# ajingu/RealSenseCalibration

Hardware: AMD Instinct MI355X
Metric: LM iterations/sec (64 cams x 100k pts point model; + final reprojection RMS px) (higher is better)
Workload: dtype f64

## Files before the change

realsensecalibration_amd/csrc/ba_schur_plan.hpp:

```cpp
#pragma once
#include <algorithm>
#include <climits>
#include <cstddef>
#include <cstdint>
#include <vector>

namespace rsba {

#define RSBA_TG 16
#define RSBA_MAX_STAGES 32
#ifndef RSBA_CHUNK
#define RSBA_CHUNK 512
#endif
#define RSBA_CW (RSBA_CHUNK / 64)
#define RSBA_GRP 8
#define RSBA_GRP_SMALL 4
#define RSBA_SELF_SETS 6
#define RSBA_DIRECT_GROUPS 4
#define RSBA_HIT_NONE 0xffffffffu
#define RSBA_CHOL_MAXN 384
#define RSBA_PB 32
#define RSBA_PLD (RSBA_PB + 1)
#define RSBA_CT 64
#define RSBA_BSM_BPG 3
// ... 20 lines not shown
    for (int I = J + 2; I < nrt && (int)first.size() < extra; ++I) { first.push_back(I << 8 | J); taken[(size_t)I * nrt + J] = 1; }
  for (int J = nrt - 1; J >= 0 && (int)last.size() < (int)first.size(); --J)
    for (int I = nrt - 1; I >= J && (int)last.size() < (int)first.size(); --I)
      if (!taken[(size_t)I * nrt + J]) { last.push_back(I << 8 | J); taken[(size_t)I * nrt + J] = 1; }
  order = first;
  for (int I = 0; I < nrt; ++I) for (int J = 0; J <= I; ++J) if (!taken[(size_t)I * nrt + J]) order.push_back(I << 8 | J);
  order.insert(order.end(), last.begin(), last.end());
  return order;
}

struct SchurSeg {
  int ga, gb, word_begin, word_end, self;
  int tile, grp, grp_seg0, grp_nseg, tile_grp0, tile_ngrp, stage, stage_ntiles, nred, index, pad2;
};

struct SchurPlanSwitches {
  static constexpr int kUnset = INT_MIN;
  int seg_per_cu = kUnset;
  int seg_target = kUnset;
  bool sparse_pairs = true;
  int balance = 1;
  bool balance_parity = true;
  int red_delay = 250;
  static SchurPlanSwitches FromEnv();
};

struct PointLayout {
  std::vector<int> ptr;
  std::vector<int> cam;
  std::vector<double> u, v;
// ... 39 lines not shown
```

realsensecalibration_amd/csrc/ba_schur_tiled.hpp:

```cpp
#pragma once
#include <type_traits>
#include <hip/hip_runtime.h>

#include <vector>

#include "ba_point_kernels.hpp"
#include "ba_schur_plan.hpp"

struct rsba_solver;

namespace rsba {

class KernelTimer;

#define RSBA_READY_ALLDIAG 40
#define RSBA_READY_SOLVED 41
#define RSBA_READY_STARTED 42
#define RSBA_PRIO(p) __builtin_amdgcn_s_setprio(p)
#ifndef RSBA_RESIDENT
#define RSBA_RESIDENT 0
#endif
#if RSBA_RESIDENT
#define RSBA_PRIO_HITS(stage) do { if ((stage) == 0) RSBA_PRIO(2); else if ((stage) == 1) RSBA_PRIO(1); else RSBA_PRIO(0); } while (0)
#else
// ... 30 lines not shown
  int ntiles = 0;
  double* ptdata = nullptr;
  double* partial = nullptr;
  double* grp_sum = nullptr;
  int* tree_error = nullptr;
  int self_arrivals = 0;
  int* error_flag = nullptr;
  int* grp_flag = nullptr;
  int epoch = 0;
  int* sync_cnt = nullptr;
  int nsync = 0, nblocks = 0;
  int* ready = nullptr;
  int* block_seg = nullptr;
  SchurSeg* segs_ordered = nullptr;
  unsigned ticket_base = 0;
  SchurSeg* segs_ordered_self = nullptr;
  int* small_flag = nullptr;
  int nblocks_self = 0;
  int ngrp = 0;
  double* block_scal = nullptr;
  int* cam_prefix = nullptr;
  int* cam_ptr = nullptr;
  int* cm_pos = nullptr;
  double* sq_cm2[2] = {nullptr, nullptr};
  double* lin2[2] = {nullptr, nullptr};
  bool has_first_order = false;
  SchurSeg* segs_ordered_first = nullptr;
  bool lin_valid = false;
  bool pt_valid = false;
  int pt_state = -1, scal_blocks = 0;
// ... 304 lines not shown
      for (int i = 0; i < NV; ++i) v[i] = (v[i] + x0[i]) + x1[i];
    }
  }
  for (; q < n; ++q) {
    const double* p0 = in + (size_t)q * RSBA_PART * 256;
#pragma unroll
    for (int i = 0; i < NV; ++i) v[i] += p0[i * 256];
  }
}

__device__ __forceinline__ bool SingleSegmentGroup(const SchurSeg& sg) { return sg.grp_nseg == 1 && sg.nred != 0; }
__device__ __forceinline__ double* SegmentOut(const SchurSeg& sg, double* __restrict__ partial, double* __restrict__ grp_sum, int seg_index) {
  return SingleSegmentGroup(sg) ? grp_sum + (size_t)sg.grp * RSBA_PART * 256 : partial + (size_t)seg_index * RSBA_PART * 256;
}

template <int NV>
__device__ __forceinline__ bool GroupReduce(const SchurSeg& sg, const double* __restrict__ partial, double* __restrict__ grp_sum,
                                            int* __restrict__ sync_cnt, int ngrp, double* v, int* __restrict__ grp_flag, int epoch) {
  __shared__ int s_last;
  const int tid = OpaqueTid();
  __builtin_amdgcn_s_waitcnt(0);
  __syncthreads();
  if (SingleSegmentGroup(sg)) {
    if (tid == 0) __hip_atomic_store(&grp_flag[sg.grp], epoch, __ATOMIC_RELAXED, __HIP_MEMORY_SCOPE_AGENT);
    return false;
  }
  if (tid == 0) s_last = __hip_atomic_fetch_add(&sync_cnt[sg.grp], 1, __ATOMIC_RELAXED, __HIP_MEMORY_SCOPE_AGENT) == sg.grp_nseg - 1;
  __syncthreads();
  if (!s_last) return false;
  __builtin_amdgcn_fence(__ATOMIC_ACQUIRE, "agent");
  TreeSum<NV>(partial + (size_t)sg.grp_seg0 * RSBA_PART * 256 + tid, sg.grp_nseg, v);
  double* gs = grp_sum + (size_t)sg.grp * RSBA_PART * 256 + tid;
#pragma unroll
  for (int i = 0; i < NV; ++i) __hip_atomic_store(&gs[i * 256], v[i], __ATOMIC_RELAXED, __HIP_MEMORY_SCOPE_AGENT);
  if (tid == 0) __hip_atomic_store(&sync_cnt[sg.grp], 0, __ATOMIC_RELAXED, __HIP_MEMORY_SCOPE_AGENT);
  __builtin_amdgcn_s_waitcnt(0);
  __syncthreads();
  if (tid == 0) {
    __hip_atomic_store(&grp_flag[sg.grp], epoch, __ATOMIC_RELAXED, __HIP_MEMORY_SCOPE_AGENT);
    s_last = sg.nred == 0 && __hip_atomic_fetch_add(&sync_cnt[ngrp + sg.tile], 1, __ATOMIC_RELAXED, __HIP_MEMORY_SCOPE_AGENT) == sg.tile_ngrp - 1;
  }
  __syncthreads();
  if (sg.nred != 0 || !s_last) return false;
  if (tid == 0) __hip_atomic_store(&sync_cnt[ngrp + sg.tile], 0, __ATOMIC_RELAXED, __HIP_MEMORY_SCOPE_AGENT);
// ... 176 lines not shown
  const double* __restrict__ block_scal;
  double* __restrict__ gmax_p;
  int* tree_error;
  int* ticket;
  unsigned ticket_base;
  int total;
  int* grp_flag;
  int epoch;
  long long* trace;
  long long* wg_trace;
  const unsigned* __restrict__ hits;
  const unsigned* __restrict__ hit_off;
  const int* __restrict__ hit_trips;
};

template <bool kLoss, bool kSmall>
__device__ __forceinline__ void PairSegment(const SchurArgs& a, const SchurSeg& sg, int seg_index, int ticket, double* pt, unsigned long long (*mk)[RSBA_CW], double* sc) {
  const int C = a.C, P = a.P, nwords = a.nwords;
  const double* __restrict__ camc = a.camc;
  const unsigned long long* __restrict__ cam_mask = a.cam_mask;
  const double* __restrict__ ptdata = a.ptdata;
  const int* __restrict__ cam_prefix = a.cam_prefix;
  const int* __restrict__ cam_ptr = a.cam_ptr;
  const double* __restrict__ sq_cm = a.sq_cm;
  double* __restrict__ partial = a.partial;
  const int tid = OpaqueTid();
  const bool diag_tile = sg.ga == sg.gb;
  const int dt = diag_tile ? (tid & 127) : tid;
  const int pr = diag_tile ? (dt < 120 ? kDiagPair[dt] : 0) : tid;
  const int ia = pr >> 4, ib = pr & 15;
  const int cam_a = RSBA_TG * sg.ga + ia, cam_b = RSBA_TG * sg.gb + ib;
  const bool live = cam_a < C && cam_b < C && (!diag_tile || dt < 120);
  const int w0 = diag_tile ? (tid >> 7) : 0, wstep = diag_tile ? 2 : 1;
  double scv[2];
#pragma unroll
  for (int u = 0; u < 2; ++u) {
    const int i = tid + 256 * u;
    const int row = i / RSBA_SC_STRIDE, e = i - row * RSBA_SC_STRIDE;
    const int cam = row < RSBA_TG ? RSBA_TG * sg.ga + row : RSBA_TG * sg.gb + (row - RSBA_TG);
    const double* cc = camc + (size_t)(cam < C ? cam : 0) * CC_STRIDE;
    const int src = e < 9 ? CC_R + e : (e < 12 ? CC_T + e - 9 : (e == 12 ? CC_FX : (e == 13 ? CC_FY : CC_SMALL)));
    scv[u] = e < 15 ? cc[src] : 0.0;
  }
  const double* ca = sc + ia * RSBA_SC_STRIDE;
  const double* cb = sc + (RSBA_TG + ib) * RSBA_SC_STRIDE;
  {
    const int wb = sg.word_begin;
    const int nwc = min(RSBA_CW, sg.word_end - wb);
    const int j0 = wb * 64;
    const int np = max(0, min(nwc * 64, P - j0));
    static_assert(RSBA_PT_STRIDE == 12, "six 16-byte pieces a record");
    constexpr int kPtPerThread = RSBA_CHUNK * 6 / 256;
    double2 pv[kPtPerThread];
    const double2* __restrict__ src2 = reinterpret_cast<const double2*>(ptdata + (size_t)j0 * RSBA_PT_STRIDE);
#pragma unroll
    for (int u = 0; u < kPtPerThread; ++u) { const int i = tid + 256 * u; pv[u] = i < np * 6 ? src2[i] : make_double2(0.0, 0.0); }
    unsigned long long mv;
    {
      const int row = tid >> 3, w = tid & 7;
      const int cam = row < RSBA_TG ? RSBA_TG * sg.ga + row : RSBA_TG * sg.gb + (row - RSBA_TG);
      mv = (cam < C && w < nwc) ? cam_mask[(size_t)cam * nwords + (size_t)wb + w] : 0ull;
    }
    sc[tid] = scv[0]; sc[tid + 256] = scv[1];
    PtLdsCursor pc(tid);
#pragma unroll
    for (int u = 0; u < kPtPerThread; ++u) { const int i = tid + 256 * u; if (i < np * 6) reinterpret_cast<double2*>(pt)[pc.a] = pv[u]; pc.Next(); }
    if ((tid & 7) < RSBA_CW) mk[tid >> 3][tid & 7] = mv;
    __syncthreads();
  }
  double acc[36];
#pragma unroll
  for (int i = 0; i < 36; ++i) acc[i] = 0.0;

  for (int wb = sg.word_begin; wb < sg.word_end; wb += RSBA_CW) {
    const int nwc = min(RSBA_CW, sg.word_end - wb);
    if (wb != sg.word_begin) {
      const int j0 = wb * 64;
      const int np = max(0, min(nwc * 64, P - j0));
      __syncthreads();
      { PtLdsCursor pc(tid); const double2* __restrict__ src2 = reinterpret_cast<const double2*>(ptdata + (size_t)j0 * RSBA_PT_STRIDE);
        for (int i = tid; i < np * 6; i += 256) { reinterpret_cast<double2*>(pt)[pc.a] = src2[i]; pc.Next(); } }
      {
// ... 28 lines not shown
    RSBA_PRIO(3);
  }
  if (diag_tile) {
    __syncthreads();
    if (tid >= 128 && dt < 120) {
#pragma unroll
      for (int i = 0; i < 36; ++i) pt[i * 128 + dt] = acc[i];
    }
    __syncthreads();
    if (tid < 120) {
#pragma unroll
      for (int i = 0; i < 36; ++i) acc[i] += pt[i * 128 + tid];
    }
  }
  double* out = SegmentOut(sg, partial, a.grp_sum, seg_index);
  if (!diag_tile || tid < 120) {
#pragma unroll
    for (int i = 0; i < 36; ++i) __hip_atomic_store(&out[i * 256 + pr], acc[i], __ATOMIC_RELAXED, __HIP_MEMORY_SCOPE_AGENT);
  }
  if (a.wg_trace && tid == 0) a.wg_trace[3 * ticket + 2] = wall_clock64();
  double v[36];
  if (!GroupReduce<36>(sg, partial, a.grp_sum, a.sync_cnt, a.ngrp, v, a.grp_flag, a.epoch)) return;
  FinishPairSlot(C, sg.ga, sg.gb, tid, v, camc, a.red, a.L, a.cam_free);
  if (!StageArrive(sg, a.sync_cnt, a.ngrp, a.ntiles, a.tag != 0)) return;
  if (tid == 0 && a.tag) PublishStage(a.ready + 1 + sg.stage, a.tag);
  if (a.trace && tid == 0 && sg.stage < 7) a.trace[17 + sg.stage] = wall_clock64();
}

template <bool kLoss, bool kSmall>
__device__ __forceinline__ void PairSegmentSparse(const SchurArgs& a, const SchurSeg& sg, int seg_index, int ticket, double* pt, double* sc) {
  const int C = a.C;
  const double* __restrict__ camc = a.camc;
  const double* __restrict__ ptdata = a.ptdata;
  const double* __restrict__ sq_cm = a.sq_cm;
  double* __restrict__ partial = a.partial;
// ... 56 lines not shown
      for (int i = 0; i < 36; ++i) pt[i * 128 + dt] = acc[i];
    }
    __syncthreads();
    if (tid < 120) {
#pragma unroll
      for (int i = 0; i < 36; ++i) acc[i] += pt[i * 128 + tid];
    }
  }
  double* out = SegmentOut(sg, partial, a.grp_sum, seg_index);
  if (!diag_tile || tid < 120) {
#pragma unroll
    for (int i = 0; i < 36; ++i) __hip_atomic_store(&out[i * 256 + pr], acc[i], __ATOMIC_RELAXED, __HIP_MEMORY_SCOPE_AGENT);
  }
  if (a.wg_trace && tid == 0) a.wg_trace[3 * ticket + 2] = wall_clock64();
  double v[36];
  if (!GroupReduce<36>(sg, partial, a.grp_sum, a.sync_cnt, a.ngrp, v, a.grp_flag, a.epoch)) return;
  FinishPairSlot(C, sg.ga, sg.gb, tid, v, camc, a.red, a.L, a.cam_free);
  if (!StageArrive(sg, a.sync_cnt, a.ngrp, a.ntiles, a.tag != 0)) return;
  if (tid == 0 && a.tag) PublishStage(a.ready + 1 + sg.stage, a.tag);
  if (a.trace && tid == 0 && sg.stage < 7) a.trace[17 + sg.stage] = wall_clock64();
}

template <bool kLoss>
__device__ __forceinline__ void SelfSegment(const SchurArgs& a, const SchurSeg& sg, int seg_index, int ticket, double* pt, unsigned long long (*mk)[RSBA_CW],
                                            unsigned short (*lst)[RSBA_CHUNK], int* cnt) {
  const int C = a.C, P = a.P, nwords = a.nwords;
  const double* __restrict__ camc = a.camc;
  const unsigned long long* __restrict__ cam_mask = a.cam_mask;
  const double* __restrict__ ptdata = a.ptdata;
  const int* __restrict__ cam_prefix = a.cam_prefix;
  const int* __restrict__ cam_ptr = a.cam_ptr;
  const double* __restrict__ sq_cm = a.sq_cm;
  const double* __restrict__ u_cm = a.u_cm;
  const double* __restrict__ v_cm = a.v_cm;
  double* __restrict__ partial = a.partial;
  const int tid = OpaqueTid(), ia = tid >> 4, ib = tid & 15;
  const int cam_a = RSBA_TG * sg.ga + ia;
  const bool live = cam_a < C;
  const double* cca = camc + (size_t)(live ? cam_a : 0) * CC_STRIDE;
  SideConst A;
  LoadSide(cca, A);
  const double ppx = cca[CC_PPX], ppy = cca[CC_PPY];
  const int obs0 = live ? cam_ptr[cam_a] : 0;
  double acc[RSBA_PART];
#pragma unroll
  for (int i = 0; i < RSBA_PART; ++i) acc[i] = 0.0;
  for (int wb = sg.word_begin; wb < sg.word_end; wb += RSBA_CW) {
    const int nwc = min(RSBA_CW, sg.word_end - wb);
    const int j0 = wb * 64;
    const int np = max(0, min(nwc * 64, P - j0));
    static_assert(RSBA_PT_STRIDE == 12, "six 16-byte pieces a record");
    constexpr int kPtPerThread = RSBA_CHUNK * 6 / 256;
    double2 pv[kPtPerThread];
    const double2* __restrict__ src2 = reinterpret_cast<const double2*>(ptdata + (size_t)j0 * RSBA_PT_STRIDE);
#pragma unroll
    for (int u = 0; u < kPtPerThread; ++u) { const int i = tid + 256 * u; pv[u] = i < np * 6 ? src2[i] : make_double2(0.0, 0.0); }
    unsigned long long mv = 0ull;
    if (tid < RSBA_TG * 8) {
      const int row = tid >> 3, w = tid & 7;
      const int cam = RSBA_TG * sg.ga + row;
      mv = (cam < C && w < nwc) ? cam_mask[(size_t)cam * nwords + (size_t)wb + w] : 0ull;
    }
    const int obs_chunk_pre = live ? cam_prefix[(size_t)cam_a * nwords + wb] : 0;
    __syncthreads();
    PtLdsCursor pc(tid);
#pragma unroll
    for (int u = 0; u < kPtPerThread; ++u) { const int i = tid + 256 * u; if (i < np * 6) reinterpret_cast<double2*>(pt)[pc.a] = pv[u]; pc.Next(); }
    if (tid < RSBA_TG * 8 && (tid & 7) < RSBA_CW) mk[tid >> 3][tid & 7] = mv;
    __syncthreads();
    {
      const int row = tid >> 4, j = tid & 15, w = j >> 1, half = j & 1;
      int base = 0;
#pragma unroll
      for (int x = 0; x < RSBA_CW; ++x) base += x < w ? __popcll(mk[row][x]) : 0;
      const unsigned long long m = w < RSBA_CW ? mk[row][w] : 0ull;
      unsigned int my = half ? (unsigned int)(m >> 32) : (unsigned int)m;
      if (half) base += __popc((unsigned int)m);
      if (j == 2 * RSBA_CW - 1) cnt[row] = base + __popc(my);
      const int p0 = w * 64 + half * 32;
      while (my != 0u) {
        const int b = __ffs((int)my) - 1;
        my &= my - 1u;
        lst[row][base++] = (unsigned short)(p0 + b);
// ... 37 lines not shown
        }
      }
      acc[21] = Fma2(e0[0], e0[0], e1[0], e1[0], acc[21]); acc[22] = Fma2(e0[0], e0[1], e1[0], e1[1], acc[22]); acc[23] = Fma2(e0[0], e0[2], e1[0], e1[2], acc[23]);
      acc[24] = Fma2(e0[1], e0[1], e1[1], e1[1], acc[24]); acc[25] = Fma2(e0[1], e0[2], e1[1], e1[2], acc[25]); acc[26] = Fma2(e0[2], e0[2], e1[2], e1[2], acc[26]);
      acc[27] = fma(e0[3], e0[3], acc[27]); acc[28] = fma(e1[4], e1[4], acc[28]); acc[29] = Fma2(e0[5], e0[5], e1[5], e1[5], acc[29]);
      const double f0 = n0[0] * pd[9] + n0[1] * pd[10] + n0[2] * pd[11];
      const double f1 = n1[0] * pd[9] + n1[1] * pd[10] + n1[2] * pd[11];
#pragma unroll
      for (int p = 0; p < 6; ++p) {
        if (p == 3) { acc[33] = fma(e0[3], r0, acc[33]); acc[39] = fma(e0[3], f0, acc[39]); }
        else if (p == 4) { acc[34] = fma(e1[4], r1, acc[34]); acc[40] = fma(e1[4], f1, acc[40]); }
        else { acc[30 + p] = Fma2(e0[p], r0, e1[p], r1, acc[30 + p]); acc[36 + p] = Fma2(e0[p], f0, e1[p], f1, acc[36 + p]); }
      }
    }
    RSBA_PRIO(3);
  }
  double* out = SegmentOut(sg, partial, a.grp_sum, seg_index);
#pragma unroll
  for (int i = 0; i < RSBA_PART; ++i) __hip_atomic_store(&out[i * 256 + tid], acc[i], __ATOMIC_RELAXED, __HIP_MEMORY_SCOPE_AGENT);
  if (a.wg_trace && tid == 0) a.wg_trace[3 * ticket + 2] = wall_clock64();
  double v[RSBA_PART];
  if (!GroupReduce<RSBA_PART>(sg, partial, a.grp_sum, a.sync_cnt, a.ngrp, v, a.grp_flag, a.epoch)) return;
  FinishSelfSlot(C, sg.ga, v, camc, a.red, a.L, a.cam_free);
  if (sg.ga == a.last_group) FinishLinearize(a.nblocks_pp, a.block_scal, a.red, a.L, a.gmax_p, reinterpret_cast<double (*)[4]>(pt));
  if (a.self_only) return;
  const bool stage_done = StageArrive(sg, a.sync_cnt, a.ngrp, a.ntiles, a.tag != 0);
  if (a.all_self && a.tag && tid == 0) SelfTileArrive(a.sync_cnt, a.ngrp, a.ntiles, a.self_arrivals, a.ready, a.tag);
  if (!stage_done) return;
  if (tid == 0 && a.tag) PublishStage(a.ready + 1 + sg.stage, a.tag);
  if (a.trace && tid == 0 && sg.stage < 7) a.trace[17 + sg.stage] = wall_clock64();
}

template <int NC, typename CompOf>
__device__ __forceinline__ bool ReduceGroupsInOrder(const SchurArgs& a, const SchurSeg& sg, const double* __restrict__ in, CompOf comp, double* v, int nc_live) {
  __shared__ int s_run;
// ... 198 lines not shown
  const bool stage_done = StageArrive(sg, a.sync_cnt, a.ngrp, a.ntiles, lin && a.tag != 0);
  if (a.all_self && a.tag && tid == 0) SelfTileArrive(a.sync_cnt, a.ngrp, a.ntiles, a.self_arrivals, a.ready, a.tag);
  if (!stage_done) return;
  if (tid == 0 && a.tag) PublishStage(a.ready + 1 + sg.stage, a.tag);
  if (a.trace && tid == 0 && sg.stage < 7) a.trace[17 + sg.stage] = wall_clock64();
}

__device__ __forceinline__ void ReducerSegment(const SchurArgs& a, const SchurSeg& sg, int ticket, char* lds) {
  if (sg.self == 2) ReducerQuadrant(a, sg, ticket);
  else ReducerSelfSet(a, sg, ticket, lds);
}

#define RSBA_PAIRS_MASKED 0
#define RSBA_PAIRS_SPARSE 1
#define RSBA_SCHUR_LDS_BYTES (RSBA_CHUNK * RSBA_PT_LDS * 8 + 2048 + 4096 + 2 * RSBA_TG * RSBA_CHUNK + 96)
template <bool kLoss, int kMode>
__global__ void __launch_bounds__(256, 2)
k_schur_tiles(int* __restrict__ ticket_p, unsigned ticket_base, int total, const int* __restrict__ small_flag_p, const SchurSeg* __restrict__ segs_p, SchurArgs a) {
  __shared__ __attribute__((aligned(16))) char lds_raw[RSBA_SCHUR_LDS_BYTES];
  static_assert(RSBA_CHUNK * RSBA_PT_LDS * 8 + 2048 + 4096 + 2 * RSBA_TG * RSBA_CHUNK + 64 <= RSBA_SCHUR_LDS_BYTES, "LDS carve");
  static_assert(RSBA_CHUNK != 512 || 2 * (RSBA_SCHUR_LDS_BYTES + 256) <= 160 * 1024, "two workgroups per CU");
  constexpr bool kSparse = kMode == RSBA_PAIRS_SPARSE;
  constexpr bool kResident = kSparse || RSBA_RESIDENT != 0;
  double* pt = reinterpret_cast<double*>(lds_raw);
  unsigned long long (*mk)[RSBA_CW] = reinterpret_cast<unsigned long long (*)[RSBA_CW]>(lds_raw + RSBA_CHUNK * RSBA_PT_LDS * 8);
  double* sc = reinterpret_cast<double*>(lds_raw + RSBA_CHUNK * RSBA_PT_LDS * 8 + 2048);
  unsigned short (*lst)[RSBA_CHUNK] = reinterpret_cast<unsigned short (*)[RSBA_CHUNK]>(lds_raw + RSBA_CHUNK * RSBA_PT_LDS * 8 + 2048 + 4096);
  int* cnt = reinterpret_cast<int*>(lds_raw + RSBA_CHUNK * RSBA_PT_LDS * 8 + 2048 + 4096 + 2 * RSBA_TG * RSBA_CHUNK);
  __shared__ int s_ticket, s_small;
  RSBA_PRIO(3);
  if (threadIdx.x == 0) s_small = __hip_atomic_load(small_flag_p, __ATOMIC_RELAXED, __HIP_MEMORY_SCOPE_AGENT);
  for (;;) {
    if (threadIdx.x == 0) s_ticket = (int)((unsigned)__hip_atomic_fetch_add(ticket_p, 1, __ATOMIC_RELAXED, __HIP_MEMORY_SCOPE_AGENT) - ticket_base);
    __syncthreads();
    const int b = __builtin_amdgcn_readfirstlane(s_ticket);
    if (kResident && b >= total) break;
    const SchurSeg sg = LoadSeg(segs_p + b);
    const int seg_index = sg.index;
    if (a.trace && b == 0 && threadIdx.x == 0) a.trace[24] = wall_clock64();
    if (a.wg_trace && threadIdx.x == 0) a.wg_trace[3 * b] = wall_clock64();
    if (sg.self >= 2) ReducerSegment(a, sg, b, lds_raw);
    else if (sg.self) SelfSegment<kLoss>(a, sg, seg_index, b, pt, mk, lst, cnt);
    else {
      if (kSparse) {
        if (s_small) PairSegmentSparse<kLoss, true>(a, sg, seg_index, b, pt, sc);
        else PairSegmentSparse<kLoss, false>(a, sg, seg_index, b, pt, sc);
      } else if (s_small) PairSegment<kLoss, true>(a, sg, seg_index, b, pt, mk, sc);
      else PairSegment<kLoss, false>(a, sg, seg_index, b, pt, mk, sc);
    }
    if (a.wg_trace && threadIdx.x == 0) a.wg_trace[3 * b + 1] = wall_clock64();
    if (!kResident) break;
    __syncthreads();
  }
}


__global__ void __launch_bounds__(64) k_wait_stage(const int* __restrict__ flag, int tag, int* __restrict__ error) {
  if (threadIdx.x == 0) {
    const long long t0 = wall_clock64();
    while (__hip_atomic_load(flag, __ATOMIC_RELAXED, __HIP_MEMORY_SCOPE_AGENT) != tag) {
      __builtin_amdgcn_s_sleep(8);
      if (wall_clock64() - t0 > 10 * RSBA_STALL_TICKS) { __hip_atomic_store(error, 1, __ATOMIC_RELAXED, __HIP_MEMORY_SCOPE_AGENT); break; }
    }
  }
}
__global__ void __launch_bounds__(64) k_set_flag(int* __restrict__ flag, int tag) {
// ... 5 lines not shown
```

realsensecalibration_amd/csrc/ba_solver.hip:

```cpp
#include <hip/hip_runtime.h>
#include <dlfcn.h>

#include <algorithm>
#include <atomic>
#include <chrono>
#include <cmath>
#include <cstdio>
#include <cstdlib>
#include <cstring>
#include <functional>
#include <map>
#include <mutex>
#include <string>
#include <vector>

#include "ba_comm.hpp"
#include "ba_covariance.hpp"
#include "ba_evaluate.hpp"
#include "ba_evaluate_jacobian.hpp"
#include "ba_marker_kernels.hpp"
#include "ba_marker_pose.hpp"
#include "ba_marker_schur.hpp"
#include "ba_resection.hpp"
#include "ba_rig_start_plan.hpp"
// ... 692 lines not shown
  T.Begin("k_point_damp", st);
  k_point_damp<<<grid_pp, 256, 0, st>>>(P, s->pts[x], s->scale_p, lin2[x], ptdata, block_scal, C, s->camc[x], small_flag, ip, s->trace);
  T.End(st);
  pt_valid = true; pt_state = x; pt_radius = ip.radius; scal_blocks = grid_pp;
}

static void LaunchPointSide(TiledSchur& ts, rsba_solver* s, const IterParams& ip, KernelTimer& T, hipStream_t st) {
  RoctxRange rr("K1+K2 point side: residuals, cost, point blocks (or their damping)");
  if (ts.lin_valid && !ip.first) {
    if (!(ts.pt_valid && ts.pt_state == s->cur && ts.pt_radius == ip.radius)) ts.LaunchPointDamp(s, ip, T, st);
  } else {
    ts.LaunchPointPass(s, ip, T, st);
  }
}

static int SchurGrid(int entries, bool sparse, int resident_spare) {
  if (RSBA_RESIDENT != 0 && !sparse) return std::min(entries, std::max(1, 2 * DeviceCUs() - resident_spare));
  return sparse ? std::min(entries, 2 * DeviceCUs()) : entries;
}

__global__ void __launch_bounds__(256) k_pack_lower(int n, const double* __restrict__ red, RedLayout L, double* __restrict__ tri, int sym_full) {
  const size_t nt = (size_t)n * (n + 1) / 2, total = nt + 3 * (size_t)n + 8;
  for (size_t k = (size_t)blockIdx.x * blockDim.x + threadIdx.x; k < total; k += (size_t)gridDim.x * blockDim.x) {
    if (k >= nt) { tri[k] = red[L.gc() + (k - nt)]; continue; }
    size_t i = (size_t)((sqrt(8.0 * (double)k + 1.0) - 1.0) * 0.5);
    while (i * (i + 1) / 2 > k) --i;
    while ((i + 1) * (i + 2) / 2 <= k) ++i;
    const size_t j = k - i * (i + 1) / 2;
    tri[k] = sym_full ? red[L.S() + i * (size_t)n + j] : red[L.S() + j * (size_t)n + i];
  }
}
__global__ void __launch_bounds__(256) k_unpack_lower(int n, const double* __restrict__ tri, double* __restrict__ red, RedLayout L) {
  const size_t nn = (size_t)n * n, nt = (size_t)n * (n + 1) / 2, total = nn + 3 * (size_t)n + 8;
  for (size_t k = (size_t)blockIdx.x * blockDim.x + threadIdx.x; k < total; k += (size_t)gridDim.x * blockDim.x) {
    if (k >= nn) { red[L.gc() + (k - nn)] = tri[nt + (k - nn)]; continue; }
    const size_t i = k / n, j = k - i * n, hi = i > j ? i : j, lo = i > j ? j : i;
    red[L.S() + k] = tri[hi * (hi + 1) / 2 + lo];
  }
}

static void LaunchSchurInstance(const SchurArgs& a, int grid, bool loss, hipStream_t st) {
#define RSBA_LAUNCH_SCHUR(LOSS, MODE) k_schur_tiles<LOSS, MODE><<<grid, 256, 0, st>>>(a.ticket, a.ticket_base, a.total, a.small_flag, a.segs_ordered, a)
  if (a.hits != nullptr) { if (loss) RSBA_LAUNCH_SCHUR(true, RSBA_PAIRS_SPARSE); else RSBA_LAUNCH_SCHUR(false, RSBA_PAIRS_SPARSE); }
  else if (loss) RSBA_LAUNCH_SCHUR(true, RSBA_PAIRS_MASKED);
  else RSBA_LAUNCH_SCHUR(false, RSBA_PAIRS_MASKED);
#undef RSBA_LAUNCH_SCHUR
}

static SchurArgs MakeSchurArgs(TiledSchur& ts, rsba_solver* s, int tag) {
  const int x = s->cur;
  SchurArgs a;
  a.C = ts.C; a.P = ts.P; a.nwords = ts.nwords; a.camc = s->camc[x]; a.cam_free = s->cam_free; a.segs = ts.segs; a.cam_mask = ts.cam_mask; a.ptdata = ts.ptdata;
  a.cam_prefix = ts.cam_prefix; a.cam_ptr = ts.cam_ptr; a.sq_cm = ts.sq_cm2[x]; a.u_cm = ts.u_cm; a.v_cm = ts.v_cm; a.partial = ts.partial;
  a.grp_sum = ts.grp_sum; a.sync_cnt = ts.sync_cnt; a.ngrp = ts.ngrp; a.ntiles = ts.ntiles; a.segs_ordered = ts.segs_ordered; a.small_flag = ts.small_flag; a.last_group = ts.ngroups - 1;
  a.tree_error = ts.error_flag ? ts.error_flag : ts.tree_error; a.ticket = ts.tree_error + 1;
  a.ready = ts.ready; a.tag = tag; a.self_only = 0; a.red = s->red; a.L = s->L; a.nblocks_pp = ts.scal_blocks; a.block_scal = ts.block_scal; a.gmax_p = s->gmax;
  a.trace = s->trace; a.wg_trace = s->wg_trace;
  a.grp_flag = ts.grp_flag; a.epoch = ++ts.epoch;
  a.hits = ts.hits; a.hit_off = ts.hit_off; a.hit_trips = ts.hit_trips;
  a.all_self = 0; a.self_arrivals = ts.self_arrivals;
  return a;
}

void TiledSchur::LaunchTiles(rsba_solver* s, const IterParams& ip, KernelTimer& T, hipStream_t st, int tag, bool first_staged) {
  RoctxRange rr("K2+K3 camera-side rows + Schur elimination into the reduced system");
  SchurArgs a = MakeSchurArgs(*this, s, tag);
  if (first_staged) { a.segs_ordered = segs_ordered_first; a.all_self = 1; }
  const bool sparse = a.hits != nullptr;
  const int grid = SchurGrid(nblocks, sparse, s->sw.resident_spare);
  a.total = nblocks; a.ticket_base = ticket_base; ticket_base += (unsigned)(nblocks + ((sparse || RSBA_RESIDENT != 0) ? grid : 0));
  T.Begin("k_schur_tiles", st);
  LaunchSchurInstance(a, grid, ip.huber_delta != 0.0, st);
  T.End(st);
}

void TiledSchur::LaunchSelfOnly(rsba_solver* s, const IterParams& ip, KernelTimer& T, hipStream_t st) {
  RoctxRange rr("K2 camera gradient only (self tiles)");
  SchurArgs a = MakeSchurArgs(*this, s, 0);
  a.segs_ordered = segs_ordered_self; a.self_only = 1; a.trace = nullptr; a.wg_trace = nullptr;
  const int grid = SchurGrid(nblocks_self, false, s->sw.resident_spare);
  a.total = nblocks_self; a.ticket_base = ticket_base; ticket_base += (unsigned)(nblocks_self + (RSBA_RESIDENT != 0 ? grid : 0));
  T.Begin("k_schur_tiles(self only)", st);
  a.hits = nullptr;
  LaunchSchurInstance(a, grid, ip.huber_delta != 0.0, st);
  T.End(st);
}

int TiledSchur::Launch(rsba_solver* s, const IterParams& ip, KernelTimer& T) {
  hipStream_t st = s->stream;
  LaunchPointSide(*this, s, ip, T, st);
  LaunchTiles(s, ip, T, st, 0);
  return RSBA_OK;
}

static void TraceRingDump(rsba_solver* s) {
  if (!s->trace_ring || !s->trace_base || s->trace_ring_first_tag == 0) return;
  if (hipStreamSynchronize(s->stream) != hipSuccess) return;
  std::vector<long long> h((size_t)64 * s->trace_ring);
  if (hipMemcpy(h.data(), s->trace_base, h.size() * sizeof(long long), hipMemcpyDeviceToHost) != hipSuccess) return;
// ... 1536 lines not shown
  return RSBA_OK;
}

int rsba_solver_create(rsba_problem* p, const rsba_options* o, rsba_solver** out) {
  if (!p || !out) return RSBA_ERR_ARG;
  if (rsba::DeviceCount() <= 0) return RSBA_ERR_NO_DEVICE;
  rsba_options opt;
  if (o) opt = *o; else rsba_options_default(&opt);
  if (opt.world_size > 1 && (!opt.comm_unique_id || opt.rank < 0 || opt.rank >= opt.world_size)) return RSBA_ERR_ARG;
  if (opt.world_size > 1 && p->model != RSBA_MODEL_POINTS) return RSBA_ERR_UNSUPPORTED;
  if (!(opt.max_solver_time_in_seconds >= 0.0)) return RSBA_ERR_ARG;
  const auto t0 = std::chrono::steady_clock::now();
  rsba_solver* s = new rsba_solver();
  s->prob = p; s->opt = opt;
  s->sw = StepSwitches::FromEnv();
  if (opt.device >= 0) { if (hipSetDevice(opt.device) != hipSuccess) { delete s; return RSBA_ERR_HIP; } }
  if (hipGetDevice(&s->device) != hipSuccess) { delete s; return RSBA_ERR_HIP; }
  if (opt.stream) s->stream = (hipStream_t)opt.stream;
  else { if (hipStreamCreateWithFlags(&s->stream, hipStreamNonBlocking) != hipSuccess) { delete s; return RSBA_ERR_HIP; } s->own_stream = true; }
  s->timer.Enable(opt.profile_kernels);
  if (opt.profile_kernels) s->timer.Reserve(256);
  int rc = RSBA_OK;
  if (opt.world_size > 1 || getenv("RSBA_FORCE_COMM")) {
    const size_t nc6 = 6 * (size_t)std::max(p->num_cameras, 1);
    s->comm = opt.world_size > 1 && rsba::LoopbackComm::IsLoopbackId(opt.comm_unique_id)
                  ? rsba::LoopbackComm::Create(opt.world_size, opt.rank, opt.comm_unique_id)
              : opt.world_size > 1 && rsba::ShmComm::IsShmId(opt.comm_unique_id)
                  ? rsba::ShmComm::Create(opt.world_size, opt.rank, opt.comm_unique_id, (nc6 * nc6 + 3 * nc6 + 64) * sizeof(double))
                  : rsba::RcclComm::Create(opt.world_size, opt.rank, opt.comm_unique_id);
    if (!s->comm) { rsba::FreeSolver(s); return RSBA_ERR_COMM; }
// ... 815 lines not shown
```

Before: 2956.

## Let Schur workgroups take multiple segments and prefetch the next chunk ahead

Adds an optional multi-entry mode where each Schur workgroup draws several segment tickets in turn. It prefetches the next segment's first point chunk and camera data into registers before the group-arrive atomic, then stages them into LDS when the group is not the last arriver. The self-segment loop is also restructured to load the next chunk after computing the current one, so global loads overlap compute. The multi-entry count defaults to 1, so on the default path only the restructured loads and the arrive/stage-ahead logic change. Staging registers raise register pressure, and the ticket accounting becomes more complex.

```diff
diff --git a/realsensecalibration_amd/csrc/ba_schur_plan.hpp b/realsensecalibration_amd/csrc/ba_schur_plan.hpp
--- a/realsensecalibration_amd/csrc/ba_schur_plan.hpp
+++ b/realsensecalibration_amd/csrc/ba_schur_plan.hpp
@@ -58,6 +58,22 @@
   int tile, grp, grp_seg0, grp_nseg, tile_grp0, tile_ngrp, stage, stage_ntiles, nred, index, pad2;
 };
 
+#define RSBA_SCHUR_ENTRIES_MAX 8
+#ifndef RSBA_SCHUR_ENTRIES_DEFAULT
+#define RSBA_SCHUR_ENTRIES_DEFAULT 1
+#endif
+struct SchurLaunchShape {
+  int grid;
+  unsigned draws;
+};
+inline int ClampSchurEntries(int entries) { return entries < 1 ? 1 : (entries > RSBA_SCHUR_ENTRIES_MAX ? RSBA_SCHUR_ENTRIES_MAX : entries); }
+inline SchurLaunchShape SchurEntriesShape(int total, int entries) {
+  SchurLaunchShape s;
+  s.grid = (total + entries - 1) / entries;
+  s.draws = (unsigned)s.grid * (unsigned)entries;
+  return s;
+}
+
 struct SchurPlanSwitches {
   static constexpr int kUnset = INT_MIN;
   int seg_per_cu = kUnset;
diff --git a/realsensecalibration_amd/csrc/ba_schur_tiled.hpp b/realsensecalibration_amd/csrc/ba_schur_tiled.hpp
--- a/realsensecalibration_amd/csrc/ba_schur_tiled.hpp
+++ b/realsensecalibration_amd/csrc/ba_schur_tiled.hpp
@@ -68,6 +68,7 @@
   int* block_seg = nullptr;
   SchurSeg* segs_ordered = nullptr;
   unsigned ticket_base = 0;
+  int entries = RSBA_SCHUR_ENTRIES_DEFAULT;
   SchurSeg* segs_ordered_self = nullptr;
   int* small_flag = nullptr;
   int nblocks_self = 0;
@@ -402,9 +403,29 @@
   return SingleSegmentGroup(sg) ? grp_sum + (size_t)sg.grp * RSBA_PART * 256 : partial + (size_t)seg_index * RSBA_PART * 256;
 }
 
-template <int NV>
-__device__ __forceinline__ bool GroupReduce(const SchurSeg& sg, const double* __restrict__ partial, double* __restrict__ grp_sum,
-                                            int* __restrict__ sync_cnt, int ngrp, double* v, int* __restrict__ grp_flag, int epoch) {
+struct SchurStaged {
+  double2 pv[RSBA_CHUNK * 6 / 256];
+  unsigned long long mv;
+  double scv[2];
+  int pre;
+};
+
+struct SchurAhead {
+  int left;
+  int b;
+  int in_lds;
+  SchurSeg sg;
+  int* __restrict__ ticket_p; unsigned ticket_base; int total; const SchurSeg* __restrict__ segs_p;
+  int* s_ticket;
+};
+__device__ __forceinline__ void ClearAhead(SchurAhead& ah) {
+  ah.b = -1; ah.in_lds = 0;
+#define RSBA_F(f) ah.sg.f = 0
+  RSBA_F(ga); RSBA_F(gb); RSBA_F(word_begin); RSBA_F(word_end); RSBA_F(self); RSBA_F(tile); RSBA_F(grp); RSBA_F(grp_seg0); RSBA_F(grp_nseg);
+  RSBA_F(tile_grp0); RSBA_F(tile_ngrp); RSBA_F(stage); RSBA_F(stage_ntiles); RSBA_F(nred); RSBA_F(index); RSBA_F(pad2);
+#undef RSBA_F
+}
+__device__ __forceinline__ bool GroupArrive(const SchurSeg& sg, int* __restrict__ sync_cnt, int* __restrict__ grp_flag, int epoch) {
   __shared__ int s_last;
   const int tid = OpaqueTid();
   __builtin_amdgcn_s_waitcnt(0);
@@ -415,7 +436,13 @@
   }
   if (tid == 0) s_last = __hip_atomic_fetch_add(&sync_cnt[sg.grp], 1, __ATOMIC_RELAXED, __HIP_MEMORY_SCOPE_AGENT) == sg.grp_nseg - 1;
   __syncthreads();
-  if (!s_last) return false;
+  return s_last != 0;
+}
+template <int NV>
+__device__ __forceinline__ bool GroupReduce(const SchurSeg& sg, const double* __restrict__ partial, double* __restrict__ grp_sum,
+                                            int* __restrict__ sync_cnt, int ngrp, double* v, int* __restrict__ grp_flag, int epoch) {
+  __shared__ int s_last;
+  const int tid = OpaqueTid();
   __builtin_amdgcn_fence(__ATOMIC_ACQUIRE, "agent");
   TreeSum<NV>(partial + (size_t)sg.grp_seg0 * RSBA_PART * 256 + tid, sg.grp_nseg, v);
   double* gs = grp_sum + (size_t)sg.grp * RSBA_PART * 256 + tid;
@@ -622,8 +649,95 @@
   const int* __restrict__ hit_trips;
 };
 
+__device__ __forceinline__ void LoadChunk(const SchurArgs& a, const SchurSeg& sg, int wb, SchurStaged& st) {
+  const int tid = OpaqueTid();
+  const int C = a.C, nwords = a.nwords;
+  const int nwc = min(RSBA_CW, sg.word_end - wb);
+  const int j0 = wb * 64;
+  const int np = max(0, min(nwc * 64, a.P - j0));
+  static_assert(RSBA_PT_STRIDE == 12, "six 16-byte pieces a record");
+  constexpr int kPtPerThread = RSBA_CHUNK * 6 / 256;
+  const double2* __restrict__ src2 = reinterpret_cast<const double2*>(a.ptdata + (size_t)j0 * RSBA_PT_STRIDE);
+#pragma unroll
+  for (int u = 0; u < kPtPerThread; ++u) { const int i = tid + 256 * u; st.pv[u] = i < np * 6 ? src2[i] : make_double2(0.0, 0.0); }
+  const int row = tid >> 3, w = tid & 7;
+  if (sg.self) {
+    const int cam = RSBA_TG * sg.ga + row;
+    st.mv = (row < RSBA_TG && cam < C && w < nwc) ? a.cam_mask[(size_t)cam * nwords + (size_t)wb + w] : 0ull;
+    const int cam_a = RSBA_TG * sg.ga + (tid >> 4);
+    st.pre = cam_a < C ? a.cam_prefix[(size_t)cam_a * nwords + wb] : 0;
+  } else {
+    const int cam = row < RSBA_TG ? RSBA_TG * sg.ga + row : RSBA_TG * sg.gb + (row - RSBA_TG);
+    st.mv = (cam < C && w < nwc) ? a.cam_mask[(size_t)cam * nwords + (size_t)wb + w] : 0ull;
+    st.pre = 0;
+  }
+}
+__device__ __forceinline__ void LoadFirstChunk(const SchurArgs& a, const SchurSeg& sg, SchurStaged& st) {
+  const int tid = OpaqueTid();
+  st.scv[0] = 0.0; st.scv[1] = 0.0;
+  if (!sg.self) {
+#pragma unroll
+    for (int u = 0; u < 2; ++u) {
+      const int i = tid + 256 * u;
+      const int row = i / RSBA_SC_STRIDE, e = i - row * RSBA_SC_STRIDE;
+      const int cam = row < RSBA_TG ? RSBA_TG * sg.ga + row : RSBA_TG * sg.gb + (row - RSBA_TG);
+      const double* cc = a.camc + (size_t)(cam < a.C ? cam : 0) * CC_STRIDE;
+      const int src = e < 9 ? CC_R + e : (e < 12 ? CC_T + e - 9 : (e == 12 ? CC_FX : (e == 13 ? CC_FY : CC_SMALL)));
+      st.scv[u] = e < 15 ? cc[src] : 0.0;
+    }
+  }
+  LoadChunk(a, sg, sg.word_begin, st);
+}
+
+__device__ __forceinline__ void StoreChunkLds(const SchurArgs& a, const SchurSeg& sg, int wb, const SchurStaged& st, bool first, double* pt,
+                                              unsigned long long (*mk)[RSBA_CW], double* sc) {
+  const int tid = OpaqueTid();
+  const int nwc = min(RSBA_CW, sg.word_end - wb);
+  const int np = max(0, min(nwc * 64, a.P - wb * 64));
+  constexpr int kPtPerThread = RSBA_CHUNK * 6 / 256;
+  if (first && !sg.self) { sc[tid] = st.scv[0]; sc[tid + 256] = st.scv[1]; }
+  PtLdsCursor pc(tid);
+#pragma unroll
+  for (int u = 0; u < kPtPerThread; ++u) { const int i = tid + 256 * u; if (i < np * 6) reinterpret_cast<double2*>(pt)[pc.a] = st.pv[u]; pc.Next(); }
+  if ((sg.self == 0 || tid < RSBA_TG * 8) && (tid & 7) < RSBA_CW) mk[tid >> 3][tid & 7] = st.mv;
+}
+
+__device__ __forceinline__ unsigned IssueDraw(const SchurAhead& ah) {
+  unsigned t = 0u;
+  if (ah.left > 0 && OpaqueTid() == 0) t = (unsigned)__hip_atomic_fetch_add(ah.ticket_p, 1, __ATOMIC_RELAXED, __HIP_MEMORY_SCOPE_AGENT);
+  return t;
+}
+__device__ __forceinline__ bool DrawAhead(SchurAhead& ah, unsigned drawn) {
+  if (ah.left <= 0) return false;
+  --ah.left;
+  if (OpaqueTid() == 0) *ah.s_ticket = (int)(drawn - ah.ticket_base);
+  __syncthreads();
+  ah.b = __builtin_amdgcn_readfirstlane(*ah.s_ticket);
+  if (ah.b >= ah.total) return false;
+  ah.sg = LoadSeg(ah.segs_p + ah.b);
+  return ah.sg.self < 2;
+}
+__device__ __forceinline__ bool ArriveAndStageAhead(const SchurArgs& a, const SchurSeg& sg, SchurAhead& ah, unsigned drawn, double* pt,
+                                                    unsigned long long (*mk)[RSBA_CW], double* sc) {
+  if (!DrawAhead(ah, drawn)) return GroupArrive(sg, a.sync_cnt, a.grp_flag, a.epoch);
+  SchurStaged st;
+  LoadFirstChunk(a, ah.sg, st);
+  __builtin_amdgcn_sched_barrier(0);
+  __builtin_amdgcn_s_waitcnt(0);
+#pragma unroll
+  for (int u = 0; u < RSBA_CHUNK * 6 / 256; ++u) { asm volatile("" : "+v"(st.pv[u].x), "+v"(st.pv[u].y)); }
+  asm volatile("" : "+v"(st.mv), "+v"(st.scv[0]), "+v"(st.scv[1]), "+v"(st.pre));
+  const bool last = GroupArrive(sg, a.sync_cnt, a.grp_flag, a.epoch);
+  if (!last) {
+    StoreChunkLds(a, ah.sg, ah.sg.word_begin, st, true, pt, mk, sc);
+    ah.in_lds = 1;
+  }
+  return last;
+}
+
 template <bool kLoss, bool kSmall>
-__device__ __forceinline__ void PairSegment(const SchurArgs& a, const SchurSeg& sg, int seg_index, int ticket, double* pt, unsigned long long (*mk)[RSBA_CW], double* sc) {
+__device__ __forceinline__ void PairSegment(const SchurArgs& a, const SchurSeg& sg, int seg_index, int ticket, double* pt, unsigned long long (*mk)[RSBA_CW], double* sc,
+                                            SchurAhead& ah) {
   const int C = a.C, P = a.P, nwords = a.nwords;
   const double* __restrict__ camc = a.camc;
   const unsigned long long* __restrict__ cam_mask = a.cam_mask;
@@ -640,40 +754,15 @@
   const int cam_a = RSBA_TG * sg.ga + ia, cam_b = RSBA_TG * sg.gb + ib;
   const bool live = cam_a < C && cam_b < C && (!diag_tile || dt < 120);
   const int w0 = diag_tile ? (tid >> 7) : 0, wstep = diag_tile ? 2 : 1;
-  double scv[2];
-#pragma unroll
-  for (int u = 0; u < 2; ++u) {
-    const int i = tid + 256 * u;
-    const int row = i / RSBA_SC_STRIDE, e = i - row * RSBA_SC_STRIDE;
-    const int cam = row < RSBA_TG ? RSBA_TG * sg.ga + row : RSBA_TG * sg.gb + (row - RSBA_TG);
-    const double* cc = camc + (size_t)(cam < C ? cam : 0) * CC_STRIDE;
-    const int src = e < 9 ? CC_R + e : (e < 12 ? CC_T + e - 9 : (e == 12 ? CC_FX : (e == 13 ? CC_FY : CC_SMALL)));
-    scv[u] = e < 15 ? cc[src] : 0.0;
-  }
   const double* ca = sc + ia * RSBA_SC_STRIDE;
   const double* cb = sc + (RSBA_TG + ib) * RSBA_SC_STRIDE;
   {
-    const int wb = sg.word_begin;
-    const int nwc = min(RSBA_CW, sg.word_end - wb);
-    const int j0 = wb * 64;
-    const int np = max(0, min(nwc * 64, P - j0));
-    static_assert(RSBA_PT_STRIDE == 12, "six 16-byte pieces a record");
-    constexpr int kPtPerThread = RSBA_CHUNK * 6 / 256;
-    double2 pv[kPtPerThread];
-    const double2* __restrict__ src2 = reinterpret_cast<const double2*>(ptdata + (size_t)j0 * RSBA_PT_STRIDE);
-#pragma unroll
-    for (int u = 0; u < kPtPerThread; ++u) { const int i = tid + 256 * u; pv[u] = i < np * 6 ? src2[i] : make_double2(0.0, 0.0); }
-    unsigned long long mv;
-    {
-      const int row = tid >> 3, w = tid & 7;
-      const int cam = row < RSBA_TG ? RSBA_TG * sg.ga + row : RSBA_TG * sg.gb + (row - RSBA_TG);
-      mv = (cam < C && w < nwc) ? cam_mask[(size_t)cam * nwords + (size_t)wb + w] : 0ull;
-    }
-    sc[tid] = scv[0]; sc[tid + 256] = scv[1];
-    PtLdsCursor pc(tid);
-#pragma unroll
-    for (int u = 0; u < kPtPerThread; ++u) { const int i = tid + 256 * u; if (i < np * 6) reinterpret_cast<double2*>(pt)[pc.a] = pv[u]; pc.Next(); }
-    if ((tid & 7) < RSBA_CW) mk[tid >> 3][tid & 7] = mv;
+    if (!ah.in_lds) {
+      SchurStaged st;
+      LoadFirstChunk(a, sg, st);
+      StoreChunkLds(a, sg, sg.word_begin, st, true, pt, mk, sc);
+    }
+    ClearAhead(ah);
     __syncthreads();
   }
   double acc[36];
@@ -732,11 +821,13 @@
     }
   }
   double* out = SegmentOut(sg, partial, a.grp_sum, seg_index);
+  const unsigned drawn = IssueDraw(ah);
   if (!diag_tile || tid < 120) {
 #pragma unroll
     for (int i = 0; i < 36; ++i) __hip_atomic_store(&out[i * 256 + pr], acc[i], __ATOMIC_RELAXED, __HIP_MEMORY_SCOPE_AGENT);
   }
   if (a.wg_trace && tid == 0) a.wg_trace[3 * ticket + 2] = wall_clock64();
+  if (!ArriveAndStageAhead(a, sg, ah, drawn, pt, mk, sc)) return;
   double v[36];
   if (!GroupReduce<36>(sg, partial, a.grp_sum, a.sync_cnt, a.ngrp, v, a.grp_flag, a.epoch)) return;
   FinishPairSlot(C, sg.ga, sg.gb, tid, v, camc, a.red, a.L, a.cam_free);
@@ -823,7 +914,7 @@
   }
   if (a.wg_trace && tid == 0) a.wg_trace[3 * ticket + 2] = wall_clock64();
   double v[36];
-  if (!GroupReduce<36>(sg, partial, a.grp_sum, a.sync_cnt, a.ngrp, v, a.grp_flag, a.epoch)) return;
+  if (!GroupArrive(sg, a.sync_cnt, a.grp_flag, a.epoch) || !GroupReduce<36>(sg, partial, a.grp_sum, a.sync_cnt, a.ngrp, v, a.grp_flag, a.epoch)) return;
   FinishPairSlot(C, sg.ga, sg.gb, tid, v, camc, a.red, a.L, a.cam_free);
   if (!StageArrive(sg, a.sync_cnt, a.ngrp, a.ntiles, a.tag != 0)) return;
   if (tid == 0 && a.tag) PublishStage(a.ready + 1 + sg.stage, a.tag);
@@ -832,12 +923,9 @@
 
 template <bool kLoss>
 __device__ __forceinline__ void SelfSegment(const SchurArgs& a, const SchurSeg& sg, int seg_index, int ticket, double* pt, unsigned long long (*mk)[RSBA_CW],
-                                            unsigned short (*lst)[RSBA_CHUNK], int* cnt) {
-  const int C = a.C, P = a.P, nwords = a.nwords;
+                                            unsigned short (*lst)[RSBA_CHUNK], int* cnt, double* sc, SchurAhead& ah) {
+  const int C = a.C, P = a.P;
   const double* __restrict__ camc = a.camc;
-  const unsigned long long* __restrict__ cam_mask = a.cam_mask;
-  const double* __restrict__ ptdata = a.ptdata;
-  const int* __restrict__ cam_prefix = a.cam_prefix;
   const int* __restrict__ cam_ptr = a.cam_ptr;
   const double* __restrict__ sq_cm = a.sq_cm;
   const double* __restrict__ u_cm = a.u_cm;
@@ -854,28 +942,18 @@
   double acc[RSBA_PART];
 #pragma unroll
   for (int i = 0; i < RSBA_PART; ++i) acc[i] = 0.0;
-  for (int wb = sg.word_begin; wb < sg.word_end; wb += RSBA_CW) {
-    const int nwc = min(RSBA_CW, sg.word_end - wb);
-    const int j0 = wb * 64;
-    const int np = max(0, min(nwc * 64, P - j0));
-    static_assert(RSBA_PT_STRIDE == 12, "six 16-byte pieces a record");
-    constexpr int kPtPerThread = RSBA_CHUNK * 6 / 256;
-    double2 pv[kPtPerThread];
-    const double2* __restrict__ src2 = reinterpret_cast<const double2*>(ptdata + (size_t)j0 * RSBA_PT_STRIDE);
-#pragma unroll
-    for (int u = 0; u < kPtPerThread; ++u) { const int i = tid + 256 * u; pv[u] = i < np * 6 ? src2[i] : make_double2(0.0, 0.0); }
-    unsigned long long mv = 0ull;
-    if (tid < RSBA_TG * 8) {
-      const int row = tid >> 3, w = tid & 7;
-      const int cam = RSBA_TG * sg.ga + row;
-      mv = (cam < C && w < nwc) ? cam_mask[(size_t)cam * nwords + (size_t)wb + w] : 0ull;
-    }
-    const int obs_chunk_pre = live ? cam_prefix[(size_t)cam_a * nwords + wb] : 0;
-    __syncthreads();
-    PtLdsCursor pc(tid);
-#pragma unroll
-    for (int u = 0; u < kPtPerThread; ++u) { const int i = tid + 256 * u; if (i < np * 6) reinterpret_cast<double2*>(pt)[pc.a] = pv[u]; pc.Next(); }
-    if (tid < RSBA_TG * 8 && (tid & 7) < RSBA_CW) mk[tid >> 3][tid & 7] = mv;
+  bool in_lds = ah.in_lds != 0;
+  ClearAhead(ah);
+  SchurStaged st;
+  if (!in_lds) LoadChunk(a, sg, sg.word_begin, st);
+  else st.pre = live ? a.cam_prefix[(size_t)cam_a * a.nwords + sg.word_begin] : 0;
+  for (int wb = sg.word_begin; wb < sg.word_end;) {
+    const int obs_chunk_pre = st.pre;
+    if (!in_lds) {
+      __syncthreads();
+      StoreChunkLds(a, sg, wb, st, false, pt, mk, nullptr);
+    }
+    in_lds = false;
     __syncthreads();
     {
       const int row = tid >> 4, j = tid & 15, w = j >> 1, half = j & 1;
@@ -943,11 +1021,16 @@
       }
     }
     RSBA_PRIO(3);
+    wb += RSBA_CW;
+    if (wb >= sg.word_end) break;
+    LoadChunk(a, sg, wb, st);
   }
   double* out = SegmentOut(sg, partial, a.grp_sum, seg_index);
+  const unsigned drawn = IssueDraw(ah);
 #pragma unroll
   for (int i = 0; i < RSBA_PART; ++i) __hip_atomic_store(&out[i * 256 + tid], acc[i], __ATOMIC_RELAXED, __HIP_MEMORY_SCOPE_AGENT);
   if (a.wg_trace && tid == 0) a.wg_trace[3 * ticket + 2] = wall_clock64();
+  if (!ArriveAndStageAhead(a, sg, ah, drawn, pt, mk, sc)) return;
   double v[RSBA_PART];
   if (!GroupReduce<RSBA_PART>(sg, partial, a.grp_sum, a.sync_cnt, a.ngrp, v, a.grp_flag, a.epoch)) return;
   FinishSelfSlot(C, sg.ga, v, camc, a.red, a.L, a.cam_free);
@@ -1176,9 +1259,9 @@
 #define RSBA_PAIRS_MASKED 0
 #define RSBA_PAIRS_SPARSE 1
 #define RSBA_SCHUR_LDS_BYTES (RSBA_CHUNK * RSBA_PT_LDS * 8 + 2048 + 4096 + 2 * RSBA_TG * RSBA_CHUNK + 96)
-template <bool kLoss, int kMode>
+template <bool kLoss, int kMode, bool kMulti = false>
 __global__ void __launch_bounds__(256, 2)
-k_schur_tiles(int* __restrict__ ticket_p, unsigned ticket_base, int total, const int* __restrict__ small_flag_p, const SchurSeg* __restrict__ segs_p, SchurArgs a) {
+k_schur_tiles(int* __restrict__ ticket_p, unsigned ticket_base, int total, int entries, const int* __restrict__ small_flag_p, const SchurSeg* __restrict__ segs_p, SchurArgs a) {
   __shared__ __attribute__((aligned(16))) char lds_raw[RSBA_SCHUR_LDS_BYTES];
   static_assert(RSBA_CHUNK * RSBA_PT_LDS * 8 + 2048 + 4096 + 2 * RSBA_TG * RSBA_CHUNK + 64 <= RSBA_SCHUR_LDS_BYTES, "LDS carve");
   static_assert(RSBA_CHUNK != 512 || 2 * (RSBA_SCHUR_LDS_BYTES + 256) <= 160 * 1024, "two workgroups per CU");
@@ -1192,26 +1275,40 @@
   __shared__ int s_ticket, s_small;
   RSBA_PRIO(3);
   if (threadIdx.x == 0) s_small = __hip_atomic_load(small_flag_p, __ATOMIC_RELAXED, __HIP_MEMORY_SCOPE_AGENT);
+  SchurAhead ah;
+  ClearAhead(ah);
+  ah.left = kResident ? 0 : (kMulti ? entries : 1);
+  ah.ticket_p = ticket_p; ah.ticket_base = ticket_base; ah.total = total; ah.segs_p = segs_p; ah.s_ticket = &s_ticket;
   for (;;) {
-    if (threadIdx.x == 0) s_ticket = (int)((unsigned)__hip_atomic_fetch_add(ticket_p, 1, __ATOMIC_RELAXED, __HIP_MEMORY_SCOPE_AGENT) - ticket_base);
-    __syncthreads();
-    const int b = __builtin_amdgcn_readfirstlane(s_ticket);
-    if (kResident && b >= total) break;
-    const SchurSeg sg = LoadSeg(segs_p + b);
+    const bool held = ah.b >= 0;
+    int b = ah.b;
+    if (!held) {
+      if (!kResident) { if (ah.left <= 0) break; --ah.left; }
+      if (threadIdx.x == 0) s_ticket = (int)((unsigned)__hip_atomic_fetch_add(ticket_p, 1, __ATOMIC_RELAXED, __HIP_MEMORY_SCOPE_AGENT) - ticket_base);
+      __syncthreads();
+      b = __builtin_amdgcn_readfirstlane(s_ticket);
+    }
+    if (b >= total) {
+      if (kResident) break;
+      ah.b = -1;
+      __syncthreads();
+      continue;
+    }
+    const SchurSeg sg = held ? ah.sg : LoadSeg(segs_p + b);
     const int seg_index = sg.index;
     if (a.trace && b == 0 && threadIdx.x == 0) a.trace[24] = wall_clock64();
     if (a.wg_trace && threadIdx.x == 0) a.wg_trace[3 * b] = wall_clock64();
-    if (sg.self >= 2) ReducerSegment(a, sg, b, lds_raw);
-    else if (sg.self) SelfSegment<kLoss>(a, sg, seg_index, b, pt, mk, lst, cnt);
+    if (sg.self >= 2) { ClearAhead(ah); ReducerSegment(a, sg, b, lds_raw); }
+    else if (sg.self) SelfSegment<kLoss>(a, sg, seg_index, b, pt, mk, lst, cnt, sc, ah);
     else {
       if (kSparse) {
         if (s_small) PairSegmentSparse<kLoss, true>(a, sg, seg_index, b, pt, sc);
         else PairSegmentSparse<kLoss, false>(a, sg, seg_index, b, pt, sc);
-      } else if (s_small) PairSegment<kLoss, true>(a, sg, seg_index, b, pt, mk, sc);
-      else PairSegment<kLoss, false>(a, sg, seg_index, b, pt, mk, sc);
+      } else if (s_small) PairSegment<kLoss, true>(a, sg, seg_index, b, pt, mk, sc, ah);
+      else PairSegment<kLoss, false>(a, sg, seg_index, b, pt, mk, sc, ah);
     }
     if (a.wg_trace && threadIdx.x == 0) a.wg_trace[3 * b + 1] = wall_clock64();
-    if (!kResident) break;
+    if (!kResident && (!kMulti || (ah.b < 0 && ah.left <= 0))) break;
     __syncthreads();
   }
 }
diff --git a/realsensecalibration_amd/csrc/ba_solver.hip b/realsensecalibration_amd/csrc/ba_solver.hip
--- a/realsensecalibration_amd/csrc/ba_solver.hip
+++ b/realsensecalibration_amd/csrc/ba_solver.hip
@@ -730,9 +730,13 @@
   }
 }
 
-static int SchurGrid(int entries, bool sparse, int resident_spare) {
-  if (RSBA_RESIDENT != 0 && !sparse) return std::min(entries, std::max(1, 2 * DeviceCUs() - resident_spare));
-  return sparse ? std::min(entries, 2 * DeviceCUs()) : entries;
+static SchurLaunchShape SchurShape(int total, bool sparse, int per_wg, int resident_spare) {
+  SchurLaunchShape shape;
+  if (RSBA_RESIDENT != 0 && !sparse) shape.grid = std::min(total, std::max(1, 2 * DeviceCUs() - resident_spare));
+  else if (sparse) shape.grid = std::min(total, 2 * DeviceCUs());
+  else return SchurEntriesShape(total, per_wg);
+  shape.draws = (unsigned)(total + shape.grid);
+  return shape;
 }
 
 __global__ void __launch_bounds__(256) k_pack_lower(int n, const double* __restrict__ red, RedLayout L, double* __restrict__ tri, int sym_full) {
@@ -755,11 +759,13 @@
   }
 }
 
-static void LaunchSchurInstance(const SchurArgs& a, int grid, bool loss, hipStream_t st) {
-#define RSBA_LAUNCH_SCHUR(LOSS, MODE) k_schur_tiles<LOSS, MODE><<<grid, 256, 0, st>>>(a.ticket, a.ticket_base, a.total, a.small_flag, a.segs_ordered, a)
-  if (a.hits != nullptr) { if (loss) RSBA_LAUNCH_SCHUR(true, RSBA_PAIRS_SPARSE); else RSBA_LAUNCH_SCHUR(false, RSBA_PAIRS_SPARSE); }
-  else if (loss) RSBA_LAUNCH_SCHUR(true, RSBA_PAIRS_MASKED);
-  else RSBA_LAUNCH_SCHUR(false, RSBA_PAIRS_MASKED);
+static void LaunchSchurInstance(const SchurArgs& a, int grid, int entries, bool loss, hipStream_t st) {
+#define RSBA_LAUNCH_SCHUR(LOSS, MODE, MULTI) k_schur_tiles<LOSS, MODE, MULTI><<<grid, 256, 0, st>>>(a.ticket, a.ticket_base, a.total, entries, a.small_flag, a.segs_ordered, a)
+  const bool multi = entries > 1 && RSBA_RESIDENT == 0;
+  if (a.hits != nullptr) { if (loss) RSBA_LAUNCH_SCHUR(true, RSBA_PAIRS_SPARSE, false); else RSBA_LAUNCH_SCHUR(false, RSBA_PAIRS_SPARSE, false); }
+  else if (multi) { if (loss) RSBA_LAUNCH_SCHUR(true, RSBA_PAIRS_MASKED, true); else RSBA_LAUNCH_SCHUR(false, RSBA_PAIRS_MASKED, true); }
+  else if (loss) RSBA_LAUNCH_SCHUR(true, RSBA_PAIRS_MASKED, false);
+  else RSBA_LAUNCH_SCHUR(false, RSBA_PAIRS_MASKED, false);
 #undef RSBA_LAUNCH_SCHUR
 }
 
@@ -783,10 +789,10 @@
   SchurArgs a = MakeSchurArgs(*this, s, tag);
   if (first_staged) { a.segs_ordered = segs_ordered_first; a.all_self = 1; }
   const bool sparse = a.hits != nullptr;
-  const int grid = SchurGrid(nblocks, sparse, s->sw.resident_spare);
-  a.total = nblocks; a.ticket_base = ticket_base; ticket_base += (unsigned)(nblocks + ((sparse || RSBA_RESIDENT != 0) ? grid : 0));
+  const SchurLaunchShape shape = SchurShape(nblocks, sparse, entries, s->sw.resident_spare);
+  a.total = nblocks; a.ticket_base = ticket_base; ticket_base += shape.draws;
   T.Begin("k_schur_tiles", st);
-  LaunchSchurInstance(a, grid, ip.huber_delta != 0.0, st);
+  LaunchSchurInstance(a, shape.grid, entries, ip.huber_delta != 0.0, st);
   T.End(st);
 }
 
@@ -794,11 +800,11 @@
   RoctxRange rr("K2 camera gradient only (self tiles)");
   SchurArgs a = MakeSchurArgs(*this, s, 0);
   a.segs_ordered = segs_ordered_self; a.self_only = 1; a.trace = nullptr; a.wg_trace = nullptr;
-  const int grid = SchurGrid(nblocks_self, false, s->sw.resident_spare);
-  a.total = nblocks_self; a.ticket_base = ticket_base; ticket_base += (unsigned)(nblocks_self + (RSBA_RESIDENT != 0 ? grid : 0));
+  const SchurLaunchShape shape = SchurShape(nblocks_self, false, entries, s->sw.resident_spare);
+  a.total = nblocks_self; a.ticket_base = ticket_base; ticket_base += shape.draws;
   T.Begin("k_schur_tiles(self only)", st);
   a.hits = nullptr;
-  LaunchSchurInstance(a, grid, ip.huber_delta != 0.0, st);
+  LaunchSchurInstance(a, shape.grid, entries, ip.huber_delta != 0.0, st);
   T.End(st);
 }
 
@@ -2365,6 +2371,7 @@
   rsba_solver* s = new rsba_solver();
   s->prob = p; s->opt = opt;
   s->sw = StepSwitches::FromEnv();
+  if (const char* e = getenv("RSBA_SCHUR_ENTRIES")) s->tiled.entries = ClampSchurEntries(atoi(e));
   if (opt.device >= 0) { if (hipSetDevice(opt.device) != hipSuccess) { delete s; return RSBA_ERR_HIP; } }
   if (hipGetDevice(&s->device) != hipSuccess) { delete s; return RSBA_ERR_HIP; }
   if (opt.stream) s->stream = (hipStream_t)opt.stream;
```

After: 2953. About the same (-0.1%).
